# vfrantc/Bayesian-Enhancement-Model

Measured on AMD Instinct MI355X. Metric: images/sec (whole node) CG_UNet N=8 Bayesian eval @256x256, higher is better.
Workload: dtype f32

## Files before the change

bayesian-enhancement-model_amd/bem/modules.py:

```python
from __future__ import annotations

import math
from typing import Optional

import torch
import torch.nn as nn

from . import autograd as ag
from . import ops
from .bayes import BayesBank, Conv2dReparameterization, EvalSampleBank, Linear2dReparameterization, SampleCtx, sampling, set_module_paths
from .native import BemNativeError


def grad_mode(m: nn.Module) -> bool:
    return m.training and torch.is_grad_enabled()


def _need_cuda(x):
    if not x.is_cuda:
        raise BemNativeError("BEM modules run on the GPU through libbem_hip.so only (no CPU fallback); "
                             "move the model and input to a HIP device")


class LayerNorm2d(nn.LayerNorm):
# ... 114 lines not shown
    return wc.reshape(4, wf.shape[0], -1), wf1 @ up_b.double(), wf2


def fold_up_fuse(up: "ConvT2x2", fuse: PwConv2d, pre: Optional[PwConv2d] = None, holder: Optional[nn.Module] = None) -> "ops.UpFuseWeights":
    if fuse.bias is not None or (pre is not None and pre.bias is not None):
        raise ValueError("fold_up_fuse: a fuse / pre layer with a bias is not folded")
    c, co = up.in_channels, up.out_channels
    if c != 2 * co or (fuse.in_channels, fuse.out_channels) != (c, co) or (pre is not None and (pre.in_channels, pre.out_channels) != (c, c)):
        raise ValueError(f"fold_up_fuse: needs up C -> C/2, fuse C -> C/2 and pre C -> C (got up {c} -> {co}, fuse {fuse.in_channels} -> "
                         f"{fuse.out_channels}" + (f", pre {pre.in_channels} -> {pre.out_channels})" if pre is not None else ")"))
    srcs = [up.weight, up.bias, fuse.weight] + ([pre.weight] if pre is not None else [])

    def prep():
        wc, bc, wf2 = compose_up_fuse(up.weight.detach(), up.bias.detach(), fuse.weight.detach(), None if pre is None else pre.weight.detach())
        return ops.UpFuseWeights(ops.pack_pw_weight(wc.float().contiguous()), ops.pack_pw_weight(wf2.float().contiguous()),
                                 bc.float().contiguous(), c)
    return ops.derived(up if holder is None else holder).get(("upfuse", pre is not None), srcs, prep)


def _out_features(m):
    return m.out_features if hasattr(m, "out_features") else m.out_channels


class gdMlp(nn.Module):
    def __init__(self, in_features, hidden_features=None, out_features=None, act_layer=nn.GELU, drop=0.0, channels_first=False):
        super().__init__()
        out_features = out_features or in_features
        hidden_features = hidden_features or in_features
        self.project_in = PwConv2d(in_features, hidden_features * 2)
        self.dwconv = DwConv2d(hidden_features * 2)
        self.project_out = PwConv2d(hidden_features, out_features)
        self.act = act_layer()

    def forward_fused(self, x, norm: LayerNorm2d):
        B, C = x.shape[0], x.shape[1]
        Hd = self.project_in.out_channels // 2
        if isinstance(self.project_in, PwConv2d) and isinstance(self.dwconv, DwConv2d) and isinstance(self.project_out, PwConv2d) \
                and ops.gdmlp_x6_supported(C, Hd):
            pi, dw, po = self.project_in, self.dwconv, self.project_out

            def prep():
                perm = ops.gate_interleave(Hd, pi.weight.device)
                bg = pi.bias.detach()[perm].contiguous() if pi.bias is not None else torch.zeros(2 * Hd, device=pi.weight.device)
                return (ops.pack_pw_weight(pi.weight.detach().reshape(2 * Hd, C)[perm].contiguous(), x6=True), bg,
                        ops.dw_gate_params10(dw.weight.detach(), None if dw.bias is None else dw.bias.detach(), Hd),
                        ops.pack_pw_weight(po.weight.detach().reshape(po.out_channels, Hd).contiguous(), x6=True),
                        None if po.bias is None else po.bias.detach().contiguous())
            Wg, bg, w10, Wo, bo = ops.derived(self).get("gdmlp_x6", [t for t in (pi.weight, pi.bias, dw.weight, dw.bias, po.weight, po.bias) if t is not None], prep)
            return ops.gdmlp_x6(x, norm.weight.detach(), norm.bias.detach(), norm.eps, Wg, bg, w10, Wo, bo, Hd)
        return self.chain(x, norm)[0]

    def chain(self, x, norm: LayerNorm2d):
        B = x.shape[0]
        Wp, b = self.project_in.gemm_weights(B)
        t2 = ops.pw_gemm(x, Wp, _out_features(self.project_in), ln=(norm.weight.detach(), norm.bias.detach()),
                         ln_eps=norm.eps, bias=b)
        w, b = self.dwconv.dw_weights(B)
        g = ops.dwconv3x3(t2, w, b, mode=2)
        Wp, b = self.project_out.gemm_weights(B)
        return ops.pw_gemm(g, Wp, _out_features(self.project_out), bias=b, res=x), t2, g


SS2D_MAX_D_STATE = 16


class SS2D(nn.Module):

    def __init__(self, d_model=96, d_state=16, ssm_ratio=2.0, dt_rank="auto", act_layer=nn.SiLU, d_conv=3,
                 conv_bias=True, dropout=0.0, bias=False, dt_min=0.001, dt_max=0.1, dt_init="random", dt_scale=1.0,
                 dt_init_floor=1e-4, initialize="v0", forward_type="v2", channel_first=False, **kwargs):
        super().__init__()
        if forward_type != "v05_noz" or not channel_first or d_conv != 3 or initialize != "v0":
            raise NotImplementedError("SS2D: only forward_type='v05_noz', channel_first, d_conv=3, init v0 are on the BEM path")
        N = int(d_state)
        if not 1 <= N <= SS2D_MAX_D_STATE:
            raise NotImplementedError(f"SS2D: d_state = {N}: the fused HIP scans take 1 <= d_state <= {SS2D_MAX_D_STATE}")
        d_inner = int(ssm_ratio * d_model)
        R = math.ceil(d_model / 16) if dt_rank == "auto" else dt_rank
        self.d_inner, self.dt_rank, self.d_state = d_inner, R, N
        self.in_proj = Linear2d(d_model, d_inner, bias=bias)
        self.act = act_layer()
        self.conv2d = DwConv2d(d_inner, bias=conv_bias)
        K = 4
        self.x_proj_weight = nn.Parameter(torch.stack([nn.Linear(d_inner, R + 2 * N, bias=False).weight.detach() for _ in range(K)], 0))
        self.out_proj = Linear2d(d_inner, d_model, bias=bias)
        std = R ** -0.5 * dt_scale
        dtw, dtb = [], []
        for _ in range(K):
            w = torch.empty(d_inner, R).uniform_(-std, std)
            dt = torch.exp(torch.rand(d_inner) * (math.log(dt_max) - math.log(dt_min)) + math.log(dt_min)).clamp(min=dt_init_floor)
            dtw.append(w)
            dtb.append(dt + torch.log(-torch.expm1(-dt)))
        self.dt_projs_weight = nn.Parameter(torch.stack(dtw, 0))
        self.dt_projs_bias = nn.Parameter(torch.stack(dtb, 0))
        self.A_logs = nn.Parameter(torch.log(torch.arange(1, N + 1, dtype=torch.float32)).view(1, -1).repeat(K * d_inner, 1).contiguous())
        self.Ds = nn.Parameter(torch.ones(K * d_inner))
        self.out_norm = LayerNorm2d(d_inner)

    def _scan_params(self):
        R = self.dt_rank

        def prep():
            xw = self.x_proj_weight.detach()
            wall = ops.pack_pw_weight(torch.cat([xw[0], xw[2], xw[1], xw[3]], 0).contiguous())
            A = -torch.exp(self.A_logs.detach().float())
            A = (A.reshape(-1) if self.d_state == 1 else A).contiguous()
            return (wall, self.dt_projs_weight.detach().contiguous(), self.dt_projs_bias.detach().contiguous(), A,
                    self.Ds.detach().float().contiguous())
        return ops.derived(self).get("scan", [self.x_proj_weight, self.dt_projs_weight, self.dt_projs_bias, self.A_logs, self.Ds], prep)

    def forward_fused(self, x, norm: LayerNorm2d, keep=False):
        B, C, H, W = x.shape
        Ci, R, N, L = self.d_inner, self.dt_rank, self.d_state, H * W
        M = R + 2 * N
        wall, dtw, dtb, A, Ds = self._scan_params()
        lnw, lnb = norm.weight.detach(), norm.bias.detach()
        rm = N == 1 and ops.ss2d_scan_rm_supported(H, W, R)
        front = not keep and (rm or N > 1) and ops.ss2d_front_supported(C, 4 * M) and Ci == C \
            and type(self.in_proj) is Linear2d and type(self.conv2d) is DwConv2d
        Wp, b = self.in_proj.gemm_weights(B)
        w, bw = self.conv2d.dw_weights(B)
        t = None
        if front:
            xc, xd = ops.ss2d_front(x, lnw, lnb, norm.eps, Wp, b, w, bw, wall, 4 * M)
        else:
            t = ops.pw_gemm(x, Wp, Ci, ln=(lnw, lnb), ln_eps=norm.eps, bias=b)
            xc = ops.dwconv3x3(t, w, bw, mode=1)
            xd = ops.pw_gemm(xc, wall, 4 * M)
        xd1 = ops.transpose_plane_slice(xd, 2 * M, 2 * M)
        xd0v, xd1v = xd.view(B, 4, M, L)[:, :2], xd1.view(B, 2, M, L)
        if rm:
            y0, y1 = ops.ss2d_scan_rm(xc, xd0v, xd1v, dtw, dtb, A, Ds)
        else:
            x0, x1 = xc.view(B, Ci, L), ops.transpose_planes(xc).view(B, Ci, L)
            if N > 1:
                y0, y1 = ops.ss2d_scan_n(x0, x1, xd0v, xd1v, dtw, dtb, A, Ds)
            else:
                y0, y1 = ops.ss2d_scan(x0, x1, xd0v, xd1v, dtw, dtb, A, Ds)
            y0, y1 = y0.view(B, Ci, H, W), ops.transpose_planes(y1.view(B, Ci, W, H))
        Wp, b = self.out_proj.gemm_weights(B)
        on = self.out_norm
        out = ops.pw_gemm(y0, Wp, _out_features(self.out_proj), x2=y1, in_mode=1,
                          ln=(on.weight.detach(), on.bias.detach()), ln_eps=on.eps, bias=b, res=x)
        return (out, (t, xc, xd, xd1, y0, y1)) if keep else out

    def forward(self, x):
        raise BemNativeError("SS2D runs fused with its VSSBlock (norm prologue + residual epilogue); call the block")


class VSSBlock(nn.Module):
    def __init__(self, hidden_dim=0, drop_path=0.0, norm_layer=LayerNorm2d, channel_first=True, ssm_d_state=16,
                 ssm_ratio=2.0, ssm_dt_rank="auto", ssm_act_layer=nn.SiLU, ssm_conv=3, ssm_conv_bias=True,
                 ssm_drop_rate=0.0, ssm_init="v0", forward_type="v2", mlp_ratio=4.0, mlp_act_layer=nn.GELU,
                 mlp_drop_rate=0.0, mlp_type="mlp", use_checkpoint=False, post_norm=False, grid_size=None, **kwargs):
        super().__init__()
        if post_norm or grid_size or drop_path or mlp_type != "gdmlp" or not channel_first:
            raise NotImplementedError("VSSBlock: only pre-norm, gdmlp, channel-first, drop_path=0 are on the BEM path")
        self.norm = LayerNorm2d(hidden_dim)
        self.op = SS2D(d_model=hidden_dim, d_state=ssm_d_state, ssm_ratio=ssm_ratio, dt_rank=ssm_dt_rank,
                       act_layer=ssm_act_layer, d_conv=ssm_conv, conv_bias=ssm_conv_bias, dropout=ssm_drop_rate,
                       initialize=ssm_init, forward_type=forward_type, channel_first=channel_first)
        self.drop_path = nn.Identity()
        self.norm2 = LayerNorm2d(hidden_dim)
        self.mlp = gdMlp(in_features=hidden_dim, hidden_features=int(hidden_dim * mlp_ratio), act_layer=mlp_act_layer,
                         drop=mlp_drop_rate, channels_first=channel_first)

    def forward(self, x):
        _need_cuda(x)
        if grad_mode(self):
            return ag.vssblock(self, x)
        x = x.contiguous()
        x = self.op.forward_fused(x, self.norm)
        return self.mlp.forward_fused(x, self.norm2)


def make_vss_level(dim, num_block, d_state, ssm_ratio, mlp_ratio, mlp_type):
    return nn.Sequential(*[VSSBlock(hidden_dim=dim, drop_path=0, norm_layer=LayerNorm2d, channel_first=True,
                                    ssm_d_state=d_state, ssm_ratio=ssm_ratio, ssm_dt_rank="auto", ssm_act_layer=nn.SiLU,
                                    ssm_conv=3, ssm_conv_bias=False, ssm_drop_rate=0, ssm_init="v0",
                                    forward_type="v05_noz", mlp_ratio=mlp_ratio, mlp_act_layer=nn.GELU,
                                    mlp_drop_rate=0.0, mlp_type=mlp_type, use_checkpoint=False, post_norm=False)
                           for _ in range(num_block)])
```

bayesian-enhancement-model_amd/bem/ops.py:

```python
from __future__ import annotations

import ctypes
import os
from inspect import signature as _signature
from functools import wraps as _wraps
from math import prod as _prod
from typing import Optional

import torch

from . import native
from .native import PwArgs, check, lib
from .tables import UIQM_WIDTH, lab_tables, niqe_gamma_table, niqe_resize_table, pil_resize_table, uiqm_resized_rows


def _stream():
    return ctypes.c_void_p(torch.cuda.current_stream().cuda_stream)


def _p(t: Optional[torch.Tensor]):
    return ctypes.c_void_p(0 if t is None else t.data_ptr())


def _chk(t: Optional[torch.Tensor], name: str, dtype=torch.float32, optional=False):
    if t is None:
        if optional:
            return
        raise ValueError(f"{name} is required")
    if not t.is_cuda:
        raise native.BemNativeError(f"{name} must be a CUDA/HIP tensor: the BEM hot path has no CPU implementation")
    if t.dtype != dtype:
        raise TypeError(f"{name} must be {dtype}, got {t.dtype}")
    if not t.is_contiguous():
        raise ValueError(f"{name} must be contiguous")


_PROF = None
_KEYS = {
    "pw_x6_res<3,2,1>": ("pw_gemm", "hbm", "pw_x6_res_kernel<3, 2, 1, false, true>",
                         lambda K, M, ln, L, mode: K <= 48 and L % 2 == 0 and mode != 1),
    "pw_x6_stream<2>": ("pw_gemm", "hbm", "pw_x6_stream_kernel<2, 2, false, true, false>",
                        lambda K, M, ln, L, mode: K > 48 and not ln and M > 32 and L % 2 == 0 and mode != 1),
    "pw_gemm": ("pw_gemm", "mfma", "pw_gemm* (all variants)", lambda K, M, ln, L, mode: True),
    "gdmlp_x6<3>": ("gdmlp_x6", "mfma_bf16", "gdmlp_x6_kernel<3, 2, 2, false>", lambda C: 32 < C <= 48),
    "gdmlp_x6<5>": ("gdmlp_x6", "mfma_bf16", "gdmlp_x6_kernel<5, 3, 1, false>", lambda C: 64 < C <= 80),
    "conv2d": ("conv2d", "mfma", "conv2d_kernel", None),
    "dwconv3x3": ("dwconv3x3", "hbm", "dwconv3x3_kernel", None),
    "ss2d_scan": ("ss2d_scan", "hbm", "ss2d_scan_kernel", None),
    "transpose_planes": ("transpose_planes", "hbm", "transpose_planes_kernel", None),
    "up_fuse": ("up_fuse", "hbm", "upfuse_x6_kernel<2>", None),
    "pw_wgrad": ("pw_wgrad_", "hbm", "wgrad_x6_kernel<2, 2> + wgrad_x6_reduce_kernel (1x1 weight gradients; wgrad_kernel<*> for L % 32 != 0)", None),
    "conv_wgrad": ("conv_wgrad_", "mfma", "wgrad_kernel<*> (dense conv weight gradients)", None),
    "ss2d_scan_bwd": ("ss2d_scan_bwd", "hbm", "ss2d_scan_bwd_kernel", None),
    "dwact_bwd": ("dwact_bwd", "hbm", "dwact_bwd_kernel", None),
    "ln_bwd": ("ln_bwd", "hbm", "ln_bwd_kernel", None),
}


def profile_start(key: str):
    global _PROF
    if key not in _KEYS:
        raise ValueError(f"profile_start: unknown key {key}; choose from {sorted(_KEYS)}")
    op, bound, symbol, pred = _KEYS[key]
    _PROF = {"kernel": op, "symbol": symbol, "bound": bound, "pred": pred, "events": [], "bytes": 0.0, "flops": 0.0}


def profile_stop():
    global _PROF
    p, _PROF = _PROF, None
    if p is None:
        return None
    torch.cuda.synchronize()
    ms = sum(s.elapsed_time(e) for s, e in p["events"])
    return {"kernel": p["symbol"], "bound": p["bound"], "launches": len(p["events"]), "ms": ms,
            "bytes": p["bytes"], "flops": p["flops"]}


# ... 405 lines not shown
    for n_, t in (("x", x), ("ln_w", ln_w), ("ln_b", ln_b), ("Wp_in", Wp_in), ("dww", dww), ("Wp_x", Wp_x)):
        _chk(t, n_)
    _chk(bias_in, "bias_in", optional=True); _chk(dwb, "dwb", optional=True)
    B, C, H, W = x.shape
    if not ss2d_front_supported(C, Mx):
        raise ValueError(f"ss2d_front: C = {C} (<= 48, % 8) / Mx = {Mx} (<= 32) not supported")
    if ln_w.numel() != C or ln_b.numel() != C or dww.numel() != 9 * C or (dwb is not None and dwb.numel() != C) or (bias_in is not None and bias_in.numel() != C):
        raise ValueError("ss2d_front: parameter shapes")
    _chk_packed1("ss2d_front", (("Wp_in", Wp_in, C, C), ("Wp_x", Wp_x, Mx, C)))
    xc = torch.empty_like(x)
    xd = torch.empty(B, Mx, H, W, device=x.device, dtype=x.dtype)
    check(lib().bem_ss2d_front_x6_f32(_p(x), _p(ln_w), _p(ln_b), float(ln_eps), _p(Wp_in), _p(bias_in), _p(dww), _p(dwb), _p(Wp_x), _p(xc), _p(xd),
                                      B, C, Mx, H, W, _stream()), "ss2d_front")
    return xc, xd


def gate_interleave(Hd, device):
    j = torch.arange(Hd // 16, device=device)[:, None, None]
    c = torch.arange(16, device=device)[None, :, None]
    s_ = torch.arange(2, device=device)[None, None, :]
    return (s_ * Hd + 16 * j + c).reshape(-1)


def gdmlp_x6_supported(C, Hd):
    return C <= 80 and Hd % 16 == 0


def dw_gate_params10(dww, dwb, Hd):
    w = dww.reshape(2, Hd, 9).permute(1, 2, 0)
    b = torch.zeros(Hd, 1, 2, device=dww.device, dtype=dww.dtype) if dwb is None else dwb.reshape(2, Hd).t().reshape(Hd, 1, 2)
    return torch.cat([w, b], 1).contiguous()


def _gdmlp_x6_cost(x, Hd, **_):
    B, C, H, W = x.shape
    return 8.0 * x.numel(), 6.0 * 2.0 * B * H * W * (2 * Hd * C + Hd * C)


@_bracket(_gdmlp_x6_cost, lambda x, **_: (x.shape[1],))
def gdmlp_x6(x, ln_w, ln_b, ln_eps, Wp_gate, bias_gate, dw10, Wp_out, bias_out, Hd):
    for n_, t in (("x", x), ("ln_w", ln_w), ("ln_b", ln_b), ("Wp_gate", Wp_gate), ("bias_gate", bias_gate), ("dw10", dw10), ("Wp_out", Wp_out)):
        _chk(t, n_)
    _chk(bias_out, "bias_out", optional=True)
    B, C, H, W = x.shape
    if not gdmlp_x6_supported(C, Hd):
        raise ValueError(f"gdmlp_x6: C = {C} (<= 80) / Hd = {Hd} (% 16) not supported")
    if tuple(dw10.shape) != (Hd, 10, 2):
        raise ValueError("gdmlp_x6: depthwise parameters must come from dw_gate_params10")
    if ln_w.numel() != C or ln_b.numel() != C or bias_gate.numel() != 2 * Hd or (bias_out is not None and bias_out.numel() != C):
        raise ValueError("gdmlp_x6: parameter shapes")
    _chk_packed1("gdmlp_x6", (("Wp_gate", Wp_gate, 2 * Hd, C), ("Wp_out", Wp_out, C, Hd)))
    out = torch.empty_like(x)
    check(lib().bem_gdmlp_x6_f32(_p(x), _p(ln_w), _p(ln_b), float(ln_eps), _p(Wp_gate), _p(bias_gate), _p(dw10), _p(Wp_out),
                                 _p(bias_out), _p(out), B, C, Hd, H, W, _stream()), "gdmlp_x6")
    return out


def _dwconv3x3_cost(x, mode, **_):
    B, Cin, H, W = x.shape
    return 4.0 * B * H * W * (Cin + (Cin // 2 if mode == 2 else Cin)), 18.0 * B * Cin * H * W


@_bracket(_dwconv3x3_cost)
def dwconv3x3(x, w, bias=None, mode=0):
    _chk(x, "x"); _chk(w, "w"); _chk(bias, "bias", optional=True)
    B, Cin, H, W = x.shape
    Cout = Cin // 2 if mode == 2 else Cin
    per_b = w.dim() == 5
    Cw = w.shape[1] if per_b else w.shape[0]
    if Cw != Cin or tuple(w.shape[-3:]) != (1, 3, 3) or (per_b and w.shape[0] != B):
        raise ValueError(f"dwconv3x3: weight {tuple(w.shape)} vs input channels {Cin}")
    bb = 0
    if bias is not None:
        if bias.shape[-1] != Cin:
            raise ValueError("dwconv3x3: bias shape")
        bb = Cin if (bias.dim() == 2 and bias.shape[0] == B and B > 1) else 0
        if bias.dim() == 2 and bias.shape[0] not in (1, B):
            raise ValueError("dwconv3x3: bias batch")
    out = torch.empty(B, Cout, H, W, device=x.device, dtype=x.dtype)
    check(lib().bem_dwconv3x3_f32(_p(x), _p(w), (Cin * 9 if per_b else 0), _p(bias), bb, _p(out), B, Cout, H, W, mode,
                                  _stream()), "dwconv3x3")
    return out


USE_CONV_MFMA = True
# ... 1151 lines not shown
```

bayesian-enhancement-model_amd/csrc/gdmlp_x6.hip:

```cpp
#include "bem_common.h"
#include "x6_tile.h"

namespace {

struct GdX {
    const float* x; const float* ln_w; const float* ln_b; float ln_eps;
    const u32x4* Wpi;
    const u32x4* Wpo;
    const float* bgi;
    const float* dw10;
    int C, Hd, H, W, NCH, tx;
};

constexpr int GD_GS = 20;

__device__ __forceinline__ float gelu_gate1(float a, float b) {
    const float t = __builtin_amdgcn_rcpf(fmaf(0.3275911f * 0.70710678118654752440f, fabsf(a), 1.f));
    float p = fmaf(1.061405429f, t, -1.453152027f);
    p = fmaf(p, t, 1.421413741f);
    p = fmaf(p, t, -0.284496736f);
    p = fmaf(p, t, 0.254829592f);
    const float e = __builtin_amdgcn_exp2f(a * a * -0.72134752044448170368f);
    const float r = fmaf(-(p * t), e, 1.f);
    const float h = 0.5f * a;
    return fmaf(h, copysignf(r, a), h) * b;
}

template <int KBM, int MTO, int WOB, bool PL2>
__global__ __launch_bounds__(256, 2) void gdmlp_x6_kernel(GdX k, const float* __restrict__ bpo, float bomul, float* __restrict__ out) {
    constexpr int NPI = 3 * KBM, NPO = 3 * MTO;
    __shared__ __attribute__((aligned(16))) f32x2 T[16 * XT_TS];
    __shared__ __attribute__((aligned(16))) float G[128 * GD_GS];
    __shared__ __attribute__((aligned(16))) u32x4 Wis[2][NPI * 64];
    __shared__ __attribute__((aligned(16))) u32x4 Wos[WOB][NPO * 64];
    __shared__ __attribute__((aligned(16))) f32x2 Bss[2][16];
    __shared__ __attribute__((aligned(16))) f32x2 DWs[2][16 * 10];
    const int lane = threadIdx.x & 63, wave = __builtin_amdgcn_readfirstlane(threadIdx.x >> 6), kh = lane >> 5, n = lane & 31;
    const int b = blockIdx.z;
    int y0, x0;
    tile_origin(k.tx, y0, x0);
    const int L = k.H * k.W;
    const float* xb = k.x + (int64_t)b * k.C * L;

    const uint32_t voff = 16 * lane;
    const uint32_t wi_lds = lds_addr(Wis), wo_lds = lds_addr(Wos), bs_lds = lds_addr(Bss), dw_lds = lds_addr(DWs);
    auto dma_in = [&](int ji, int buf) {
#pragma unroll
        for (int t = 0; t < (NPI + 3) / 4; ++t) {
            const int p = wave + 4 * t;
            if (p < NPI) glds16(k.Wpi + ((int64_t)ji * NPI + p) * 64, voff, wi_lds + (buf * NPI + p) * 1024);
        }
        if (wave == (NPI & 3)) {
            const float* src = k.dw10 + (int64_t)ji * 320;
            glds16(src, voff, dw_lds + buf * 1280);
            if (lane < 16) glds16(src + 256, voff, dw_lds + buf * 1280 + 1024);
        }
        if (wave == ((NPI + 1) & 3) && lane < 8) glds16(k.bgi + (int64_t)ji * 32, voff, bs_lds + buf * 128);
    };
    auto dma_out = [&](int jo, int buf) {
#pragma unroll
        for (int t = 0; t < (NPO + 3) / 4; ++t) {
            const int p = wave + 4 * t, mt = p / 3, li = p - 3 * mt;
            if (p < NPO) glds16(k.Wpo + (((int64_t)mt * k.NCH + jo) * 3 + li) * 64, voff, wo_lds + (buf * NPO + p) * 1024);
        }
    };
    dma_in(0, 0);

    const int oy = y0 + wave, ox = x0 + n;
    f32x16 rs[MTO];
    const bool opix = oy < k.H && ox < k.W;
    const int64_t po = (int64_t)min(oy, k.H - 1) * k.W + min(ox, k.W - 1);
    auto load_res = [&]() {
        const float* rb = xb + po;
#pragma unroll
        for (int mt = 0; mt < MTO; ++mt)
#pragma unroll
            for (int r = 0; r < 16; ++r) {
                const int row = min(acc_row(r, kh, 32 * mt), k.C - 1);
                rs[mt][r] = fmaf(bpo[row], bomul, rb[(int64_t)row * L]);
            }
    };

    u32x4 xl[2][KBM][3];
    float msk[2];
    uint32_t mbit[2];
    int hpo[2];
    {
        float lnw[KBM][8], lnb[KBM][8];
#pragma unroll
        for (int kb = 0; kb < KBM; ++kb)
#pragma unroll
            for (int e = 0; e < 8; ++e) {
                const int ch = 16 * kb + 8 * kh + e;
                const float on = ch < k.C ? 1.f : 0.f;
                lnw[kb][e] = k.ln_w[min(ch, k.C - 1)] * on;
                lnb[kb][e] = k.ln_b[min(ch, k.C - 1)] * on;
            }
        float xr[2][KBM][8];
        auto load_block = [&](int i) {
            const int hp = min((wave + 4 * i) * 32 + n, XT_TS - 1);
            hpo[i] = hp;
            const int hy = hp / XT_HW, hx = hp - hy * XT_HW;
            const int gy = y0 - 1 + hy, gx = x0 - 1 + hx;
            const bool in = hp < XT_NPH && gy >= 0 && gy < k.H && gx >= 0 && gx < k.W && (wave + 4 * i) < XT_NPB;
            msk[i] = in ? 1.f : 0.f;
            mbit[i] = in ? 0xffffffffu : 0u;
            const int off = min(max(gy, 0), k.H - 1) * k.W + min(max(gx, 0), k.W - 1);
#pragma unroll
            for (int kb = 0; kb < KBM; ++kb)
#pragma unroll
                for (int e = 0; e < 8; ++e) {
                    const int ch = 16 * kb + 8 * kh + e;
                    const float v = xb[(int64_t)min(ch, k.C - 1) * L + off];
                    xr[i][kb][e] = ch < k.C ? v : 0.f;
                }
        };
        auto norm_block = [&](int i) {
            const float inv = 1.f / (float)k.C;
            float s = 0.f;
#pragma unroll
            for (int kb = 0; kb < KBM; ++kb)
#pragma unroll
                for (int e = 0; e < 8; ++e) s += xr[i][kb][e];
            s += __shfl_xor(s, 32, 64);
            const float mean = s * inv;
            float q = 0.f;
#pragma unroll
            for (int kb = 0; kb < KBM; ++kb)
#pragma unroll
                for (int e = 0; e < 8; ++e) {
                    const float d = (16 * kb + 8 * kh + e < k.C) ? xr[i][kb][e] - mean : 0.f;
                    q = fmaf(d, d, q);
                }
            q += __shfl_xor(q, 32, 64);
            const float rstd = msk[i] / sqrtf(q * inv + k.ln_eps);
#pragma unroll
            for (int kb = 0; kb < KBM; ++kb) {
                float v[8];
#pragma unroll
                for (int e = 0; e < 8; ++e) v[e] = ((xr[i][kb][e] - mean) * rstd) * lnw[kb][e] + lnb[kb][e] * msk[i];
                split8(v, xl[i][kb][0], xl[i][kb][1], xl[i][kb][2]);
            }
        };
        if (PL2) { load_block(0); load_block(1); norm_block(0); norm_block(1); }
        else { load_block(0); norm_block(0); load_block(1); norm_block(1); }
    }

    const int wb_lds = 2 * kh * XT_HW + n;
    const int c_lo = 4 * wave;

    f32x16 oh[MTO];
#pragma unroll
    for (int mt = 0; mt < MTO; ++mt)
#pragma unroll
        for (int r = 0; r < 16; ++r) oh[mt][r] = 0.f;

    auto phase_c = [&](const u32x4* Wo) {
        const float* gp = G + (wave * 32 + n) * GD_GS + 8 * kh;
        const f32x4 ga = *reinterpret_cast<const f32x4*>(gp), gb = *reinterpret_cast<const f32x4*>(gp + 4);
        const float v[8] = {ga[0], ga[1], ga[2], ga[3], gb[0], gb[1], gb[2], gb[3]};
        u32x4 gl[3];
        split8(v, gl[0], gl[1], gl[2]);
#pragma unroll
        for (int mt = 0; mt < MTO; ++mt) {
            const u32x4* wp = Wo + mt * 192 + lane;
            const u32x4 wl[3] = {wp[0], wp[64], wp[128]};
            f32x16 lo;
#pragma unroll
            for (int r = 0; r < 16; ++r) lo[r] = 0.f;
            mac6(wl, gl, oh[mt], lo);
            oh[mt] += lo;
        }
    };

    asm volatile("s_waitcnt vmcnt(0)" ::: "memory");
    __syncthreads();

// ... 52 lines not shown
                float a0x = bias[0], a0y = bias[1], a1x = bias[0], a1y = bias[1];
#pragma unroll
                for (int ty = 0; ty < 3; ++ty)
#pragma unroll
                    for (int tx = 0; tx < 3; ++tx) {
                        const f32x2 w = wq[3 * ty + tx], u0 = win[ty][tx], u1 = win[ty + 1][tx];
                        a0x = fmaf(w[0], u0[0], a0x); a0y = fmaf(w[1], u0[1], a0y);
                        a1x = fmaf(w[0], u1[0], a1x); a1y = fmaf(w[1], u1[1], a1y);
                    }
                g[cc] = f32x2{gelu_gate1(a0x, a0y), gelu_gate1(a1x, a1y)};
            }
#pragma unroll
            for (int p = 0; p < 2; ++p)
                *reinterpret_cast<f32x4*>(G + ((2 * kh + p) * 32 + n) * GD_GS + c_lo) = f32x4{g[0][p], g[1][p], g[2][p], g[3][p]};
        }
        asm volatile("s_waitcnt vmcnt(0)" ::: "memory");
        __syncthreads();
    }
    load_res();
    phase_c(Wos[(k.NCH - 1) & (WOB - 1)]);

    if (opix) {
        float* ob = out + (int64_t)b * k.C * L + po;
#pragma unroll
        for (int mt = 0; mt < MTO; ++mt)
#pragma unroll
            for (int r = 0; r < 16; ++r) {
                const int row = acc_row(r, kh, 32 * mt);
                if (row < k.C) ob[(int64_t)row * L] = oh[mt][r] + rs[mt][r];
            }
    }
}

}

extern "C" int bem_gdmlp_x6_f32(const float* x, const float* ln_w, const float* ln_b, float ln_eps, const float* Wp_gate,
                                const float* bias_gate, const float* dw_gate10, const float* Wp_out,
                                const float* bias_out, float* out, int B, int C, int Hd, int H, int W, void* stream) {
    BEM_REQUIRE(x && ln_w && ln_b && Wp_gate && bias_gate && dw_gate10 && Wp_out && out, "gdmlp_x6: null tensor");
    BEM_REQUIRE(B >= 0 && B <= 65535 && C > 0 && C <= 80 && Hd > 0 && Hd % 16 == 0 && H > 0 && W > 0,
                "gdmlp_x6: needs C <= 80 and Hd %% 16 == 0 (got C = %d, Hd = %d)", C, Hd);
    BEM_REQUIRE((((uintptr_t)Wp_gate | (uintptr_t)Wp_out | (uintptr_t)bias_gate | (uintptr_t)dw_gate10) & 15) == 0,
                "gdmlp_x6: packed weights, bias pairs and depthwise parameters must be 16-byte aligned");
    BEM_REQUIRE(x != out, "gdmlp_x6: in-place operation is not supported (halo reads)");
    BEM_REQUIRE((int64_t)C * H * W < (1ll << 31), "gdmlp_x6: plane set too large for 32-bit offsets");
    if (B == 0) return BEM_OK;
    GdX k;
    k.x = x; k.ln_w = ln_w; k.ln_b = ln_b; k.ln_eps = ln_eps;
    k.Wpi = reinterpret_cast<const u32x4*>(Wp_gate); k.Wpo = reinterpret_cast<const u32x4*>(Wp_out); k.bgi = bias_gate;
    k.dw10 = dw_gate10;
    k.C = C; k.Hd = Hd; k.H = H; k.W = W; k.NCH = Hd / 16; k.tx = cdiv(W, XT_TW);
    const float* bpop = bias_out ? bias_out : ln_w;
    const float bomul = bias_out ? 1.f : 0.f;
    dim3 grid(k.tx * cdiv(H, XT_TH), 1, B);
    hipStream_t s = (hipStream_t)stream;
    const int KB = cdiv(C, 16);
    if (KB == 1) gdmlp_x6_kernel<1, 1, 2, false><<<grid, 256, 0, s>>>(k, bpop, bomul, out);
    else if (KB == 2) gdmlp_x6_kernel<2, 1, 2, false><<<grid, 256, 0, s>>>(k, bpop, bomul, out);
    else if (KB == 3) gdmlp_x6_kernel<3, 2, 2, false><<<grid, 256, 0, s>>>(k, bpop, bomul, out);
    else if (KB == 4) gdmlp_x6_kernel<4, 2, 2, false><<<grid, 256, 0, s>>>(k, bpop, bomul, out);
    else gdmlp_x6_kernel<5, 3, 1, false><<<grid, 256, 0, s>>>(k, bpop, bomul, out);
    return bem_check_launch("gdmlp_x6");
}
```

include/bem_hip.h:

```cpp
#ifndef BEM_HIP_H
#define BEM_HIP_H

#include <stdint.h>

#ifdef __cplusplus
extern "C" {
#endif

#define BEM_OK 0
#define BEM_ERR_INVALID 1
#define BEM_ERR_LAUNCH 2

const char* bem_last_error(void);
int bem_abi_version(void);


int bem_selective_scan_fwd_f32(const float* u, const float* delta, const float* A, const float* Bm,
                               const float* Cm, const float* D, const float* delta_bias, float* out,
                               int batch, int dim, int L, int dstate, int ngroups, int delta_softplus,
                               void* stream);

int bem_selective_scan_fwd_in16(const void* u, const void* delta, const float* A, const void* Bm, const void* Cm, const float* D,
                                const float* delta_bias, float* out, int in_dtype, int batch, int dim, int L, int dstate,
                                int ngroups, int delta_softplus, void* stream);
// ... 120 lines not shown
int bem_pad_reflect_f32(const float* x, float* out, int P, int H, int W, int Hp, int Wp, void* stream);
int bem_resize_down_f32(const float* x, float* out, int P, int Hp, int Wp, int s, void* stream);
int bem_randn_f32(float* out, int64_t n, uint64_t seed, uint64_t stream_id, const uint64_t* stream_add, void* stream);
int bem_cond_postproc_f32(const float* pred, const float* target_mean, const float* noise, float* out,
                          int Bn, int h, int w, int samples_per_image, float noise_level, void* stream);
int bem_plane_mean_f32(const float* x, float* means, int P, int Hs, int Ws, int h, int w, void* stream);
int bem_candidate_finalize_f32(const float* pred, const float* target, float* final_out, float* psnr, double* ws,
                               int Bn, int samples_per_image, int Hp, int Wp, int h, int w, int gt_mean,
                               void* stream);

int bem_select_best_f32(const float* cand, const float* psnr, int* best, float* best_psnr, float* best_img, int B, int N,
                        int64_t chw, void* stream);

int bem_ssim_f32(const float* pred, const float* target, float* ssim, double* ws, int Bn, int samples_per_image, int h, int w, void* stream);

int bem_select_scores_f32(const float* cand, const float* s1, const float* s2, float weight, int rule, int* best, float* best_s1,
                          float* best_s2, float* best_img, int B, int N, int64_t chw, void* stream);

int bem_niqe_f32(const float* final, const double* mu_pris, const double* cov_pris, const double* window, const double* gam_tab, int ntab,
                 const float* rs_wh, const int* rs_ih, int kh, const float* rs_ww, const int* rs_iw, int kw, double* scores, void* ws,
                 int64_t ws_bytes, int Bn, int h, int w, void* stream);
int64_t bem_niqe_ws_bytes(int Bn, int h, int w);

int bem_uiqm_uciqe_f32(const float* final, const int* lab_tab, const int* rs_bh, const int* rs_kh, int kh, const int* rs_bv, const int* rs_kv,
                       int kv, double* uiqm, double* uciqe, void* ws, int64_t ws_bytes, int Bn, int h, int w, int Hr, void* stream);
int64_t bem_uiqm_ws_bytes(int Bn, int h, int w, int Hr);

int bem_mc_mean_f32(const float* pred, const float* target, float* out, double* ws, int B, int N, int Hp, int Wp, int h, int w,
                    int gt_mean, void* stream);

int bem_gdmlp_x6_f32(const float* x, const float* ln_w, const float* ln_b, float ln_eps, const float* Wp_gate,
                     const float* bias_gate, const float* dw_gate10, const float* Wp_out,
                     const float* bias_out, float* out, int B, int C, int Hd, int H, int W, void* stream);

int bem_ss2d_front_x6_f32(const float* x, const float* ln_w, const float* ln_b, float ln_eps, const float* Wp_in, const float* bias_in,
                          const float* dww, const float* dwb, const float* Wp_x, float* xc, float* xd, int B, int C, int Mx, int H, int W,
                          void* stream);


int bem_l1_loss_f32(const float* pred, const float* gt, float* dpred, float* loss, double* ws, int64_t n, float weight,
                    const float* gmul, void* stream);

int bem_iwt_hamilton_bwd_f32(const float* q1w, const float* q2w, const float* dout, float* dq1w, float* dq2w, int B, int h, int w,
                             void* stream);
int bem_hamilton_bwd_f32(const float* q8, const float* dout, float* dq8, int B, int H, int W, void* stream);

int bem_pixel_unshuffle2_f32(const float* x, float* out, int B, int C, int H, int W, void* stream);

int bem_channel_sum_f32(const float* x, float* out, int B, int C, int64_t L, void* stream);
int bem_add_f32(const float* a, const float* b, float* out, int64_t n, float alpha, void* stream);

int bem_ln_bwd_f32(const float* x1, const float* x2, const float* dn, const float* gamma, const float* beta, float eps,
                   const float* dres, float* dx, float* n_out, float* dgamma, float* dbeta, int B, int C, int64_t L, void* stream);
int bem_ln_fwd_f32(const float* x1, const float* x2, const float* gamma, const float* beta, float eps, float* n_out, int B, int C,
                   int64_t L, void* stream);

int bem_dwact_bwd_f32(const float* t, const float* w, const float* bias, const float* dout, float* dpre, float* dw, float* dbias,
                      int B, int Cout, int H, int W, int mode, void* stream);

typedef struct {
    const float* dy; int64_t dy_bstride; int M;
    const float* x1; int64_t x1_bstride; int C1;
    const float* x2; int64_t x2_bstride; int C2;
    float* dw; int64_t ldw; int blk_rows; int perm[4];
    float* dbias;
    int B; int L;
// ... 87 lines not shown
```

Before: 333.2.

## Fold SS2D out-projection tail into the fused gdMlp kernel for VSS blocks

Adds a vss_back_x6 kernel variant that computes the SS2D tail (y0+y1 sum, out_norm LayerNorm, out_proj GEMM, bias and residual) inside the gdMlp one-kernel tile, including recomputation over the depthwise halo. This removes a separate pw_gemm launch and the write/read round-trip of the intermediate block output. The trade-off is redundant tail GEMM work on halo pixels, extra LDS use for the out_proj weights and more register pressure. It applies only when C <= 48 and C % 8 == 0.

After: 338.8, median of 6. +1.7%, better.

```diff
diff --git a/bayesian-enhancement-model_amd/bem/modules.py b/bayesian-enhancement-model_amd/bem/modules.py
--- a/bayesian-enhancement-model_amd/bem/modules.py
+++ b/bayesian-enhancement-model_amd/bem/modules.py
@@ -170,11 +170,14 @@
         self.project_out = PwConv2d(hidden_features, out_features)
         self.act = act_layer()
 
-    def forward_fused(self, x, norm: LayerNorm2d):
+    def fused_supported(self, C):
+        return isinstance(self.project_in, PwConv2d) and isinstance(self.dwconv, DwConv2d) and isinstance(self.project_out, PwConv2d) \
+            and ops.gdmlp_x6_supported(C, self.project_in.out_channels // 2)
+
+    def forward_fused(self, x, norm: LayerNorm2d, pre=None):
         B, C = x.shape[0], x.shape[1]
         Hd = self.project_in.out_channels // 2
-        if isinstance(self.project_in, PwConv2d) and isinstance(self.dwconv, DwConv2d) and isinstance(self.project_out, PwConv2d) \
-                and ops.gdmlp_x6_supported(C, Hd):
+        if self.fused_supported(C):
             pi, dw, po = self.project_in, self.dwconv, self.project_out
 
             def prep():
@@ -185,7 +188,9 @@
                         ops.pack_pw_weight(po.weight.detach().reshape(po.out_channels, Hd).contiguous(), x6=True),
                         None if po.bias is None else po.bias.detach().contiguous())
             Wg, bg, w10, Wo, bo = ops.derived(self).get("gdmlp_x6", [t for t in (pi.weight, pi.bias, dw.weight, dw.bias, po.weight, po.bias) if t is not None], prep)
-            return ops.gdmlp_x6(x, norm.weight.detach(), norm.bias.detach(), norm.eps, Wg, bg, w10, Wo, bo, Hd)
+            return ops.gdmlp_x6(x, norm.weight.detach(), norm.bias.detach(), norm.eps, Wg, bg, w10, Wo, bo, Hd, pre=pre)
+        if pre is not None:
+            raise BemNativeError("gdMlp: the SS2D tail can be folded into the one-kernel branch only")
         return self.chain(x, norm)[0]
 
     def chain(self, x, norm: LayerNorm2d):
@@ -247,7 +252,10 @@
                     self.Ds.detach().float().contiguous())
         return ops.derived(self).get("scan", [self.x_proj_weight, self.dt_projs_weight, self.dt_projs_bias, self.A_logs, self.Ds], prep)
 
-    def forward_fused(self, x, norm: LayerNorm2d, keep=False):
+    def tail_deferrable(self, C):
+        return type(self.out_proj) is Linear2d and self.d_inner == C
+
+    def forward_fused(self, x, norm: LayerNorm2d, keep=False, defer_tail=False):
         B, C, H, W = x.shape
         Ci, R, N, L = self.d_inner, self.dt_rank, self.d_state, H * W
         M = R + 2 * N
@@ -276,8 +284,12 @@
             else:
                 y0, y1 = ops.ss2d_scan(x0, x1, xd0v, xd1v, dtw, dtb, A, Ds)
             y0, y1 = y0.view(B, Ci, H, W), ops.transpose_planes(y1.view(B, Ci, W, H))
+        on = self.out_norm
+        if defer_tail:
+            op = self.out_proj
+            Wpp = ops.derived(self).get("vss_back", [op.weight], lambda: ops.pack_vss_back_outproj(op.weight.detach()))
+            return y0, y1, on.weight.detach(), on.bias.detach(), on.eps, Wpp, (op.bias.detach() if op.bias is not None else None)
         Wp, b = self.out_proj.gemm_weights(B)
-        on = self.out_norm
         out = ops.pw_gemm(y0, Wp, _out_features(self.out_proj), x2=y1, in_mode=1,
                           ln=(on.weight.detach(), on.bias.detach()), ln_eps=on.eps, bias=b, res=x)
         return (out, (t, xc, xd, xd1, y0, y1)) if keep else out
@@ -308,6 +320,10 @@
         if grad_mode(self):
             return ag.vssblock(self, x)
         x = x.contiguous()
+        C = x.shape[1]
+        if ops.USE_VSS_BACK and self.op.tail_deferrable(C) and self.mlp.fused_supported(C) \
+                and ops.vss_back_supported(C, self.mlp.project_in.out_channels // 2):
+            return self.mlp.forward_fused(x, self.norm2, pre=self.op.forward_fused(x, self.norm, defer_tail=True))
         x = self.op.forward_fused(x, self.norm)
         return self.mlp.forward_fused(x, self.norm2)
 
diff --git a/bayesian-enhancement-model_amd/bem/ops.py b/bayesian-enhancement-model_amd/bem/ops.py
--- a/bayesian-enhancement-model_amd/bem/ops.py
+++ b/bayesian-enhancement-model_amd/bem/ops.py
@@ -42,7 +42,7 @@
     "pw_x6_stream<2>": ("pw_gemm", "hbm", "pw_x6_stream_kernel<2, 2, false, true, false>",
                         lambda K, M, ln, L, mode: K > 48 and not ln and M > 32 and L % 2 == 0 and mode != 1),
     "pw_gemm": ("pw_gemm", "mfma", "pw_gemm* (all variants)", lambda K, M, ln, L, mode: True),
-    "gdmlp_x6<3>": ("gdmlp_x6", "mfma_bf16", "gdmlp_x6_kernel<3, 2, 2, false>", lambda C: 32 < C <= 48),
+    "gdmlp_x6<3>": ("gdmlp_x6", "mfma_bf16", "vss_back_x6_kernel<3, 2, 2> (with the SS2D tail; gdmlp_x6_kernel<3, 2, 2, false> without)", lambda C: 32 < C <= 48),
     "gdmlp_x6<5>": ("gdmlp_x6", "mfma_bf16", "gdmlp_x6_kernel<5, 3, 1, false>", lambda C: 64 < C <= 80),
     "conv2d": ("conv2d", "mfma", "conv2d_kernel", None),
     "dwconv3x3": ("dwconv3x3", "hbm", "dwconv3x3_kernel", None),
@@ -514,13 +514,44 @@
     return torch.cat([w, b], 1).contiguous()
 
 
-def _gdmlp_x6_cost(x, Hd, **_):
+USE_VSS_BACK = True
+
+
+def vss_back_supported(C, Hd):
+    return C <= 48 and C % 8 == 0 and Hd % 16 == 0
+
+
+def vss_back_rows(C):
+    KB = (C + 15) // 16
+    MT = (8 * KB + 15) // 16
+    rows = [-1] * (32 * MT)
+    for mt in range(MT):
+        for kh in range(2):
+            for r in range(16):
+                s = 16 * mt + r
+                ch = 16 * (s >> 3) + 8 * kh + (s & 7)
+                if s < 8 * KB and ch < C:
+                    rows[32 * mt + (r & 3) + 8 * (r >> 2) + 4 * kh] = ch
+    return rows
+
+
+def pack_vss_back_outproj(W):
+    C = W.shape[0]
+    rows = torch.tensor(vss_back_rows(C), device=W.device)
+    Wz = torch.cat([W, W.new_zeros(1, W.shape[1])], 0)
+    return pack_pw_weight(Wz[rows].contiguous(), x6=True)
+
+
+def _gdmlp_x6_cost(x, Hd, pre, **_):
     B, C, H, W = x.shape
-    return 8.0 * x.numel(), 6.0 * 2.0 * B * H * W * (2 * Hd * C + Hd * C)
+    nb, nf = 8.0 * x.numel(), 6.0 * 2.0 * B * H * W * (2 * Hd * C + Hd * C)
+    if pre is not None:
+        nb, nf = nb + 8.0 * x.numel(), nf + 6.0 * 2.0 * B * H * W * C * C
+    return nb, nf
 
 
 @_bracket(_gdmlp_x6_cost, lambda x, **_: (x.shape[1],))
-def gdmlp_x6(x, ln_w, ln_b, ln_eps, Wp_gate, bias_gate, dw10, Wp_out, bias_out, Hd):
+def gdmlp_x6(x, ln_w, ln_b, ln_eps, Wp_gate, bias_gate, dw10, Wp_out, bias_out, Hd, *, pre=None):
     for n_, t in (("x", x), ("ln_w", ln_w), ("ln_b", ln_b), ("Wp_gate", Wp_gate), ("bias_gate", bias_gate), ("dw10", dw10), ("Wp_out", Wp_out)):
         _chk(t, n_)
     _chk(bias_out, "bias_out", optional=True)
@@ -533,6 +564,20 @@
         raise ValueError("gdmlp_x6: parameter shapes")
     _chk_packed1("gdmlp_x6", (("Wp_gate", Wp_gate, 2 * Hd, C), ("Wp_out", Wp_out, C, Hd)))
     out = torch.empty_like(x)
+    if pre is not None:
+        y0, y1, on_w, on_b, on_eps, Wp_op, b_op = pre
+        for n_, t in (("y0", y0), ("y1", y1), ("on_w", on_w), ("on_b", on_b), ("Wp_outproj", Wp_op)):
+            _chk(t, n_)
+        _chk(b_op, "bias_outproj", optional=True)
+        if not vss_back_supported(C, Hd):
+            raise ValueError(f"gdmlp_x6 with pre: C = {C} (<= 48, % 8) not supported")
+        if y0.shape != x.shape or y1.shape != x.shape or on_w.numel() != C or on_b.numel() != C or (b_op is not None and b_op.numel() != C):
+            raise ValueError("gdmlp_x6 with pre: y0 / y1 must have the shape of x, out_norm and the out_proj bias C entries")
+        _chk_packed1("gdmlp_x6", (("Wp_outproj", Wp_op, 32 * ((8 * ((C + 15) // 16) + 15) // 16), C),))
+        check(lib().bem_vss_back_x6_f32(_p(x), _p(ln_w), _p(ln_b), float(ln_eps), _p(Wp_gate), _p(bias_gate), _p(dw10), _p(Wp_out),
+                                        _p(bias_out), _p(out), B, C, Hd, H, W, _p(y0), _p(y1), _p(on_w), _p(on_b), float(on_eps),
+                                        _p(Wp_op), _p(b_op), _stream()), "gdmlp_x6")
+        return out
     check(lib().bem_gdmlp_x6_f32(_p(x), _p(ln_w), _p(ln_b), float(ln_eps), _p(Wp_gate), _p(bias_gate), _p(dw10), _p(Wp_out),
                                  _p(bias_out), _p(out), B, C, Hd, H, W, _stream()), "gdmlp_x6")
     return out
diff --git a/bayesian-enhancement-model_amd/csrc/gdmlp_x6.hip b/bayesian-enhancement-model_amd/csrc/gdmlp_x6.hip
--- a/bayesian-enhancement-model_amd/csrc/gdmlp_x6.hip
+++ b/bayesian-enhancement-model_amd/csrc/gdmlp_x6.hip
@@ -11,6 +11,16 @@
     const float* dw10;
     int C, Hd, H, W, NCH, tx;
 };
+
+struct GdPre {
+    const float* y0; const float* y1; const float* on_w; const float* on_b; float on_eps;
+    const u32x4* Wop;
+    const float* bop; float bopmul;
+};
+
+__device__ __forceinline__ float at_byte(const float* base, uint32_t byte) {
+    return *reinterpret_cast<const float*>(reinterpret_cast<const char*>(base) + byte);
+}
 
 constexpr int GD_GS = 20;
 
@@ -26,8 +36,8 @@
     return fmaf(h, copysignf(r, a), h) * b;
 }
 
-template <int KBM, int MTO, int WOB, bool PL2>
-__global__ __launch_bounds__(256, 2) void gdmlp_x6_kernel(GdX k, const float* __restrict__ bpo, float bomul, float* __restrict__ out) {
+template <int KBM, int MTO, int WOB, bool PL2, bool PRE>
+__device__ __forceinline__ void gdmlp_x6_tile(const GdX& k, const GdPre& pre, const float* __restrict__ bpo, float bomul, float* __restrict__ out) {
     constexpr int NPI = 3 * KBM, NPO = 3 * MTO;
     __shared__ __attribute__((aligned(16))) f32x2 T[16 * XT_TS];
     __shared__ __attribute__((aligned(16))) float G[128 * GD_GS];
@@ -65,13 +75,23 @@
         }
     };
     dma_in(0, 0);
+    constexpr int MTP = (8 * KBM + 15) / 16, NPW = 3 * KBM * MTP;
+    static_assert(!PRE || NPW * 1024 <= (int)sizeof(T), "out_proj's rows must fit into T");
+    if (PRE) {
+        const uint32_t t_lds = lds_addr(T);
+#pragma unroll
+        for (int t = 0; t < (NPW + 3) / 4; ++t) {
+            const int p = wave + 4 * t;
+            if (p < NPW) glds16(pre.Wop + p * 64, voff, t_lds + p * 1024);
+        }
+    }
 
     const int oy = y0 + wave, ox = x0 + n;
     f32x16 rs[MTO];
     const bool opix = oy < k.H && ox < k.W;
     const int64_t po = (int64_t)min(oy, k.H - 1) * k.W + min(ox, k.W - 1);
     auto load_res = [&]() {
-        const float* rb = xb + po;
+        const float* rb = (PRE ? out + (int64_t)b * k.C * L : xb) + po;
 #pragma unroll
         for (int mt = 0; mt < MTO; ++mt)
 #pragma unroll
@@ -87,15 +107,31 @@
     int hpo[2];
     {
         float lnw[KBM][8], lnb[KBM][8];
-#pragma unroll
-        for (int kb = 0; kb < KBM; ++kb)
-#pragma unroll
-            for (int e = 0; e < 8; ++e) {
-                const int ch = 16 * kb + 8 * kh + e;
-                const float on = ch < k.C ? 1.f : 0.f;
-                lnw[kb][e] = k.ln_w[min(ch, k.C - 1)] * on;
-                lnb[kb][e] = k.ln_b[min(ch, k.C - 1)] * on;
-            }
+        auto load_ln = [&]() {
+#pragma unroll
+            for (int kb = 0; kb < KBM; ++kb)
+#pragma unroll
+                for (int e = 0; e < 8; ++e) {
+                    const int ch = 16 * kb + 8 * kh + e;
+                    const float on = ch < k.C ? 1.f : 0.f;
+                    lnw[kb][e] = k.ln_w[min(ch, k.C - 1)] * on;
+                    lnb[kb][e] = k.ln_b[min(ch, k.C - 1)] * on;
+                }
+        };
+        if (!PRE) load_ln();
+        auto load_ln_pre = [&]() {
+#pragma unroll
+            for (int kb = 0; kb < KBM; ++kb) {
+                const int cb = 16 * kb + 8 * kh;
+                const float on = cb < k.C ? 1.f : 0.f;
+                const uint32_t cbc = cb < k.C ? cb : 0;
+#pragma unroll
+                for (int e = 0; e < 8; ++e) {
+                    lnw[kb][e] = at_byte(k.ln_w + e, 4u * cbc) * on;
+                    lnb[kb][e] = at_byte(k.ln_b + e, 4u * cbc) * on;
+                }
+            }
+        };
         float xr[2][KBM][8];
         auto load_block = [&](int i) {
             const int hp = min((wave + 4 * i) * 32 + n, XT_TS - 1);
@@ -142,7 +178,127 @@
                 split8(v, xl[i][kb][0], xl[i][kb][1], xl[i][kb][2]);
             }
         };
-        if (PL2) { load_block(0); load_block(1); norm_block(0); norm_block(1); }
+        u32x4 yl[KBM][3];
+        const float* const y0b = pre.y0 + (int64_t)b * k.C * L;
+        const float* const y1b = pre.y1 + (int64_t)b * k.C * L;
+        const uint32_t L4 = 4u * (uint32_t)L;
+        auto tail_load = [&](int i) {
+            const int hp = min((wave + 4 * i) * 32 + n, XT_TS - 1);
+            hpo[i] = hp;
+            const int hy = hp / XT_HW, hx = hp - hy * XT_HW;
+            const int gy = y0 - 1 + hy, gx = x0 - 1 + hx;
+            const bool in = hp < XT_NPH && gy >= 0 && gy < k.H && gx >= 0 && gx < k.W && (wave + 4 * i) < XT_NPB;
+            msk[i] = in ? 1.f : 0.f;
+            mbit[i] = in ? 0xffffffffu : 0u;
+            const int off = min(max(gy, 0), k.H - 1) * k.W + min(max(gx, 0), k.W - 1);
+            float ys[KBM][8];
+#pragma unroll
+            for (int kb = 0; kb < KBM; ++kb) {
+                const int cb = 16 * kb + 8 * kh;
+                const bool von = cb < k.C;
+                const uint32_t a = 4u * (uint32_t)((von ? cb : 0) * L + off);
+#pragma unroll
+                for (int e = 0; e < 8; ++e) {
+                    const float v = at_byte(y0b, a + e * L4) + at_byte(y1b, a + e * L4);
+                    ys[kb][e] = von ? v : 0.f;
+                }
+            }
+            const float inv = 1.f / (float)k.C;
+            float s = 0.f;
+#pragma unroll
+            for (int kb = 0; kb < KBM; ++kb)
+#pragma unroll
+                for (int e = 0; e < 8; ++e) s += ys[kb][e];
+            s += __shfl_xor(s, 32, 64);
+            const float mean = s * inv;
+            float q = 0.f;
+#pragma unroll
+            for (int kb = 0; kb < KBM; ++kb)
+#pragma unroll
+                for (int e = 0; e < 8; ++e) {
+                    const float d = (16 * kb + 8 * kh < k.C) ? ys[kb][e] - mean : 0.f;
+                    q = fmaf(d, d, q);
+                }
+            q += __shfl_xor(q, 32, 64);
+            const float rstd = 1.f / sqrtf(q * inv + pre.on_eps);
+#pragma unroll
+            for (int kb = 0; kb < KBM; ++kb) {
+                const int cb = 16 * kb + 8 * kh;
+                const float on = cb < k.C ? 1.f : 0.f;
+                const uint32_t cbc = cb < k.C ? cb : 0;
+                float v[8];
+#pragma unroll
+                for (int e = 0; e < 8; ++e) v[e] = ((ys[kb][e] - mean) * rstd) * (at_byte(pre.on_w + e, 4u * cbc) * on) + at_byte(pre.on_b + e, 4u * cbc) * on;
+                split8(v, yl[kb][0], yl[kb][1], yl[kb][2]);
+            }
+        };
+        auto tail_gemm = [&](int i) {
+            const int hp = hpo[i];
+            const int hy = hp / XT_HW, hx = hp - hy * XT_HW;
+            const bool ctr = mbit[i] != 0u && hy >= 1 && hy <= XT_TH && hx >= 1 && hx <= XT_TW;
+            const int off = min(max(y0 - 1 + hy, 0), k.H - 1) * k.W + min(max(x0 - 1 + hx, 0), k.W - 1);
+            float* const ob = out + (int64_t)b * k.C * L;
+            float xv[KBM][8];
+#pragma unroll
+            for (int kb = 0; kb < KBM; ++kb) {
+                const int cb = 16 * kb + 8 * kh;
+                const uint32_t a = 4u * (uint32_t)((cb < k.C ? cb : 0) * L + off);
+#pragma unroll
+                for (int e = 0; e < 8; ++e) xv[kb][e] = at_byte(xb, a + e * L4);
+            }
+#pragma unroll
+            for (int mt = 0; mt < MTP; ++mt) {
+                f32x16 hi = zero16(), lo = zero16();
+#pragma unroll
+                for (int kb = 0; kb < KBM; ++kb) {
+                    const u32x4* wp = reinterpret_cast<const u32x4*>(T) + (mt * KBM + kb) * 192 + lane;
+                    const u32x4 wl[3] = {wp[0], wp[64], wp[128]};
+                    mac6(wl, yl[kb], hi, lo);
+                }
+#pragma unroll
+                for (int r = 0; r < 16; ++r) {
+                    const int s = 16 * mt + r, kb = s >> 3, e = s & 7, cb = 16 * kb + 8 * kh;
+                    if (s < 8 * KBM) {
+                        const float v = (hi[r] + lo[r]) + at_byte(pre.bop + e, 4u * (uint32_t)(cb < k.C ? cb : 0)) * pre.bopmul + xv[kb][e];
+                        xr[i][kb][e] = cb < k.C ? v : 0.f;
+                    }
+                }
+            }
+            if (ctr) {
+#pragma unroll
+                for (int kb = 0; kb < KBM; ++kb) {
+                    const int cb = 16 * kb + 8 * kh;
+                    if (cb < k.C) {
+                        const uint32_t a = 4u * (uint32_t)(cb * L + off);
+#pragma unroll
+                        for (int e = 0; e < 8; ++e) *reinterpret_cast<float*>(reinterpret_cast<char*>(ob) + (a + e * L4)) = xr[i][kb][e];
+                    }
+                }
+            }
+        };
+        if (PRE) {
+            tail_load(0);
+            asm volatile("s_waitcnt vmcnt(0)" ::: "memory");
+            __syncthreads();
+            __builtin_amdgcn_sched_barrier(0);
+            tail_gemm(0);
+            __builtin_amdgcn_sched_barrier(0);
+            load_ln_pre();
+            norm_block(0);
+            __builtin_amdgcn_sched_barrier(0);
+            if (wave + 4 < XT_NPB) {
+                tail_load(1);
+                __builtin_amdgcn_sched_barrier(0);
+                tail_gemm(1);
+                __builtin_amdgcn_sched_barrier(0);
+                load_ln_pre();
+                norm_block(1);
+            } else {
+                msk[1] = 0.f; mbit[1] = 0u; hpo[1] = XT_TS - 1;
+#pragma unroll
+                for (int kb = 0; kb < KBM; ++kb) xl[1][kb][0] = xl[1][kb][1] = xl[1][kb][2] = u32x4{0u, 0u, 0u, 0u};
+            }
+        } else if (PL2) { load_block(0); load_block(1); norm_block(0); norm_block(1); }
         else { load_block(0); norm_block(0); load_block(1); norm_block(1); }
     }
 
@@ -261,18 +417,34 @@
     }
 }
 
-}
-
-extern "C" int bem_gdmlp_x6_f32(const float* x, const float* ln_w, const float* ln_b, float ln_eps, const float* Wp_gate,
-                                const float* bias_gate, const float* dw_gate10, const float* Wp_out,
-                                const float* bias_out, float* out, int B, int C, int Hd, int H, int W, void* stream) {
-    BEM_REQUIRE(x && ln_w && ln_b && Wp_gate && bias_gate && dw_gate10 && Wp_out && out, "gdmlp_x6: null tensor");
+
+template <int KBM, int MTO, int WOB, bool PL2>
+__global__ __launch_bounds__(256, 2) void gdmlp_x6_kernel(GdX k, const float* __restrict__ bpo, float bomul, float* __restrict__ out) {
+    gdmlp_x6_tile<KBM, MTO, WOB, PL2, false>(k, GdPre{}, bpo, bomul, out);
+}
+
+template <int KBM, int MTO, int WOB>
+__global__ __launch_bounds__(256, 2) void vss_back_x6_kernel(GdX k, GdPre pre, const float* __restrict__ bpo, float bomul, float* __restrict__ out) {
+    gdmlp_x6_tile<KBM, MTO, WOB, false, true>(k, pre, bpo, bomul, out);
+}
+
+int gd_launch(const char* op, const float* x, const float* ln_w, const float* ln_b, float ln_eps, const float* Wp_gate, const float* bias_gate,
+              const float* dw_gate10, const float* Wp_out, const float* bias_out, float* out, int B, int C, int Hd, int H, int W,
+              const GdPre* pre, void* stream) {
+    BEM_REQUIRE(x && ln_w && ln_b && Wp_gate && bias_gate && dw_gate10 && Wp_out && out, "%s: null tensor", op);
     BEM_REQUIRE(B >= 0 && B <= 65535 && C > 0 && C <= 80 && Hd > 0 && Hd % 16 == 0 && H > 0 && W > 0,
-                "gdmlp_x6: needs C <= 80 and Hd %% 16 == 0 (got C = %d, Hd = %d)", C, Hd);
+                "%s: needs C <= 80 and Hd %% 16 == 0 (got C = %d, Hd = %d)", op, C, Hd);
     BEM_REQUIRE((((uintptr_t)Wp_gate | (uintptr_t)Wp_out | (uintptr_t)bias_gate | (uintptr_t)dw_gate10) & 15) == 0,
-                "gdmlp_x6: packed weights, bias pairs and depthwise parameters must be 16-byte aligned");
-    BEM_REQUIRE(x != out, "gdmlp_x6: in-place operation is not supported (halo reads)");
-    BEM_REQUIRE((int64_t)C * H * W < (1ll << 31), "gdmlp_x6: plane set too large for 32-bit offsets");
+                "%s: packed weights, bias pairs and depthwise parameters must be 16-byte aligned", op);
+    BEM_REQUIRE(x != out, "%s: in-place operation is not supported (halo reads)", op);
+    BEM_REQUIRE((int64_t)C * H * W < (1ll << 31), "%s: plane set too large for 32-bit offsets", op);
+    if (pre) {
+        BEM_REQUIRE(pre->y0 && pre->y1 && pre->on_w && pre->on_b && pre->Wop, "%s: null tensor", op);
+        BEM_REQUIRE(((uintptr_t)pre->Wop & 15) == 0, "%s: packed out_proj weights must be 16-byte aligned", op);
+        BEM_REQUIRE(out != pre->y0 && out != pre->y1, "%s: out must not be y0 or y1 (halo reads)", op);
+        BEM_REQUIRE((int64_t)C * H * W < (1ll << 30), "%s: plane set too large for 32-bit byte offsets", op);
+        BEM_REQUIRE(C % 8 == 0 && C <= 48, "%s: needs C %% 8 == 0 and C <= 48 (got C = %d)", op, C);
+    }
     if (B == 0) return BEM_OK;
     GdX k;
     k.x = x; k.ln_w = ln_w; k.ln_b = ln_b; k.ln_eps = ln_eps;
@@ -284,10 +456,36 @@
     dim3 grid(k.tx * cdiv(H, XT_TH), 1, B);
     hipStream_t s = (hipStream_t)stream;
     const int KB = cdiv(C, 16);
-    if (KB == 1) gdmlp_x6_kernel<1, 1, 2, false><<<grid, 256, 0, s>>>(k, bpop, bomul, out);
+    if (pre) {
+        if (KB == 1) vss_back_x6_kernel<1, 1, 2><<<grid, 256, 0, s>>>(k, *pre, bpop, bomul, out);
+        else if (KB == 2) vss_back_x6_kernel<2, 1, 2><<<grid, 256, 0, s>>>(k, *pre, bpop, bomul, out);
+        else vss_back_x6_kernel<3, 2, 2><<<grid, 256, 0, s>>>(k, *pre, bpop, bomul, out);
+    }
+    else if (KB == 1) gdmlp_x6_kernel<1, 1, 2, false><<<grid, 256, 0, s>>>(k, bpop, bomul, out);
     else if (KB == 2) gdmlp_x6_kernel<2, 1, 2, false><<<grid, 256, 0, s>>>(k, bpop, bomul, out);
     else if (KB == 3) gdmlp_x6_kernel<3, 2, 2, false><<<grid, 256, 0, s>>>(k, bpop, bomul, out);
     else if (KB == 4) gdmlp_x6_kernel<4, 2, 2, false><<<grid, 256, 0, s>>>(k, bpop, bomul, out);
     else gdmlp_x6_kernel<5, 3, 1, false><<<grid, 256, 0, s>>>(k, bpop, bomul, out);
-    return bem_check_launch("gdmlp_x6");
-}
+    return bem_check_launch(op);
+}
+
+}
+
+extern "C" int bem_gdmlp_x6_f32(const float* x, const float* ln_w, const float* ln_b, float ln_eps, const float* Wp_gate,
+                                const float* bias_gate, const float* dw_gate10, const float* Wp_out,
+                                const float* bias_out, float* out, int B, int C, int Hd, int H, int W, void* stream) {
+    return gd_launch("gdmlp_x6", x, ln_w, ln_b, ln_eps, Wp_gate, bias_gate, dw_gate10, Wp_out, bias_out, out, B, C, Hd, H, W, nullptr, stream);
+}
+
+extern "C" int bem_vss_back_x6_f32(const float* x, const float* ln_w, const float* ln_b, float ln_eps, const float* Wp_gate,
+                                   const float* bias_gate, const float* dw_gate10, const float* Wp_out,
+                                   const float* bias_out, float* out, int B, int C, int Hd, int H, int W,
+                                   const float* y0, const float* y1, const float* on_w, const float* on_b, float on_eps,
+                                   const float* Wp_outproj, const float* bias_outproj, void* stream) {
+    GdPre pre;
+    pre.y0 = y0; pre.y1 = y1; pre.on_w = on_w; pre.on_b = on_b; pre.on_eps = on_eps;
+    pre.Wop = reinterpret_cast<const u32x4*>(Wp_outproj);
+    pre.bop = bias_outproj ? bias_outproj : ln_w;
+    pre.bopmul = bias_outproj ? 1.f : 0.f;
+    return gd_launch("vss_back_x6", x, ln_w, ln_b, ln_eps, Wp_gate, bias_gate, dw_gate10, Wp_out, bias_out, out, B, C, Hd, H, W, &pre, stream);
+}
diff --git a/include/bem_hip.h b/include/bem_hip.h
--- a/include/bem_hip.h
+++ b/include/bem_hip.h
@@ -176,6 +176,12 @@
 int bem_gdmlp_x6_f32(const float* x, const float* ln_w, const float* ln_b, float ln_eps, const float* Wp_gate,
                      const float* bias_gate, const float* dw_gate10, const float* Wp_out,
                      const float* bias_out, float* out, int B, int C, int Hd, int H, int W, void* stream);
+
+int bem_vss_back_x6_f32(const float* x, const float* ln_w, const float* ln_b, float ln_eps, const float* Wp_gate,
+                        const float* bias_gate, const float* dw_gate10, const float* Wp_out,
+                        const float* bias_out, float* out, int B, int C, int Hd, int H, int W,
+                        const float* y0, const float* y1, const float* on_w, const float* on_b, float on_eps,
+                        const float* Wp_outproj, const float* bias_outproj, void* stream);
 
 int bem_ss2d_front_x6_f32(const float* x, const float* ln_w, const float* ln_b, float ln_eps, const float* Wp_in, const float* bias_in,
                           const float* dww, const float* dwb, const float* Wp_x, float* xc, float* xd, int B, int C, int Mx, int H, int W,
```
